# derekmetcalf/epnn

Hardware: AMD Instinct MI355X
Metric: atoms/sec (inference), QM9-sized batch (higher is better)
Workload: dtype f32; 1 GPU; qm9_like_b1024_N29; molecules_per_gpu=1024, atoms_per_gpu=18521, N=29, pairs_under_cutoff_per_gpu=72439, entry=epnn_forward_xyz_dev (coordinates in HBM), weights=decay_model_weights, parallelism=molecule-sharded x1, batches_in_flight_per_gpu=8

## Files before the change

epnn_amd/csrc/epnn_wave.hip.h:

```cpp
#pragma once
#include <type_traits>

#include "epnn_common.h"
#include "epnn_frontend.hip.h"

struct WaveArgs {
    const float *wpack;
    const float *xin;
    const float *Q;
    const int4 *wblk;
    const int *row_off;
    const int *pi, *pj, *psym;
    float *pe, *pwi, *pwj;
    float *q_out;
    float *h_out;
    int *status;
    int N, T, nx, A;
    const float *h_in;
    const float *q_in;
    const float *nm_in;
    float *gx;
    int lds_words;
    const float *xyz;
    double cut2;
// ... 112 lines not shown
#ifndef EPNN_SPLIT_VALU
__device__ __forceinline__ void w16_split3(const float (&v)[8], u32x4 &p1, u32x4 &p2, u32x4 &p3) {
    const w16_u32x2 I = w16_ident();
    f32x4 x0 = {v[0], v[1], v[2], v[3]}, x1 = {v[4], v[5], v[6], v[7]};
    p1 = w16_pack_hi(x0, x1);
    x0 = w16_rem(I, p1[0], p1[1], x0); x1 = w16_rem(I, p1[2], p1[3], x1);
    p2 = w16_pack_hi(x0, x1);
    x0 = w16_rem(I, p2[0], p2[1], x0); x1 = w16_rem(I, p2[2], p2[3], x1);
    p3 = w16_pack_hi(x0, x1);
}
#else
__device__ __forceinline__ void w16_split3(const float (&v)[8], u32x4 &p1, u32x4 &p2, u32x4 &p3) {
    float r1[8], r2[8];
#pragma unroll
    for (int s = 0; s < 8; ++s) {
        r1[s] = v[s] - __uint_as_float(__float_as_uint(v[s]) & 0xffff0000u);
        r2[s] = r1[s] - __uint_as_float(__float_as_uint(r1[s]) & 0xffff0000u);
    }
#pragma unroll
    for (int j = 0; j < 4; ++j) {
        p1[j] = __builtin_amdgcn_perm(__float_as_uint(v[2 * j + 1]), __float_as_uint(v[2 * j]), 0x07060302u);
        p2[j] = __builtin_amdgcn_perm(__float_as_uint(r1[2 * j + 1]), __float_as_uint(r1[2 * j]), 0x07060302u);
        p3[j] = __builtin_amdgcn_perm(__float_as_uint(r2[2 * j + 1]), __float_as_uint(r2[2 * j]), 0x07060302u);
    }
}
#endif
__device__ __forceinline__ void w16_mm_bf(const u32x4 (&w)[2][3], u32x4 z1, u32x4 z2, u32x4 z3, f32x4 (&d)[2]) {
#pragma unroll
    for (int rb = 0; rb < 2; ++rb) {
        d[rb] = w16_mfma_bf(w[rb][0], z3, d[rb]);
        d[rb] = w16_mfma_bf(w[rb][1], z2, d[rb]);
        d[rb] = w16_mfma_bf(w[rb][2], z1, d[rb]);
        d[rb] = w16_mfma_bf(w[rb][0], z2, d[rb]);
        d[rb] = w16_mfma_bf(w[rb][1], z1, d[rb]);
        d[rb] = w16_mfma_bf(w[rb][0], z1, d[rb]);
    }
}
#define W16_LDB(dst, off)                                                                                       \
    _Pragma("unroll") for (int rb_ = 0; rb_ < 2; ++rb_)                                                         \
        _Pragma("unroll") for (int pc_ = 0; pc_ < 3; ++pc_)                                                     \
            (dst)[rb_][pc_] = reinterpret_cast<const u32x4 *>(wp + (size_t)(unsigned)(off))[(rb_ * 3 + pc_) * 64 + lane];
__device__ __forceinline__ void w16_split3k16(f32x4 x, w16_u32x2 &p1, w16_u32x2 &p2, w16_u32x2 &p3) {
    const w16_u32x2 I = w16_ident();
    p1 = w16_pack_hi2(x);
    x = w16_rem(I, p1[0], p1[1], x);
    p2 = w16_pack_hi2(x);
    x = w16_rem(I, p2[0], p2[1], x);
    p3 = w16_pack_hi2(x);
}
__device__ __forceinline__ void w16_mm_bfk16(const w16_u32x2 (&w)[2][3], const w16_u32x2 (&z)[3], f32x4 (&d)[2]) {
#pragma unroll
    for (int rb = 0; rb < 2; ++rb) {
        d[rb] = w16_rem(w[rb][0], z[2][0], z[2][1], d[rb]);
        d[rb] = w16_rem(w[rb][1], z[1][0], z[1][1], d[rb]);
        d[rb] = w16_rem(w[rb][2], z[0][0], z[0][1], d[rb]);
        d[rb] = w16_rem(w[rb][0], z[1][0], z[1][1], d[rb]);
        d[rb] = w16_rem(w[rb][1], z[0][0], z[0][1], d[rb]);
        d[rb] = w16_rem(w[rb][0], z[0][0], z[0][1], d[rb]);
    }
}
#define W16_LDB16(dst, off)                                                                                     \
    _Pragma("unroll") for (int rb_ = 0; rb_ < 2; ++rb_)                                                         \
        _Pragma("unroll") for (int pc_ = 0; pc_ < 3; ++pc_)                                                     \
            (dst)[rb_][pc_] = reinterpret_cast<const w16_u32x2 *>(wp + (size_t)(unsigned)(off))[(rb_ * 3 + pc_) * 64 + lane];
__device__ __forceinline__ f32x4 w16_relu(f32x4 v) {
    return f32x4{fmaxf(v[0], 0.f), fmaxf(v[1], 0.f), fmaxf(v[2], 0.f), fmaxf(v[3], 0.f)};
}
__device__ __forceinline__ float w16_sumq(float v) {
    const auto a = __builtin_amdgcn_permlane16_swap(__float_as_uint(v), __float_as_uint(v), false, false);
    const float s = __uint_as_float(a[0]) + __uint_as_float(a[1]);
    const auto b = __builtin_amdgcn_permlane32_swap(__float_as_uint(s), __float_as_uint(s), false, false);
    return __uint_as_float(b[0]) + __uint_as_float(b[1]);
}
__device__ __forceinline__ f32x4 w16_ld(const float *p) { return *reinterpret_cast<const f32x4 *>(p); }
__device__ __forceinline__ void w16_st(float *p, f32x4 v) { *reinterpret_cast<f32x4 *>(p) = v; }

typedef __attribute__((address_space(3))) const f32x4 w16_lds_cf4;
typedef __attribute__((address_space(3))) const unsigned short w16_lds_cu16;
__device__ __forceinline__ unsigned w16_lds_addr(const void *p) { return (unsigned)(size_t)(__attribute__((address_space(3))) const char *)p; }
__device__ __forceinline__ f32x4 w16_lds_ld4(unsigned a) { return *(w16_lds_cf4 *)(size_t)a; }
__device__ __forceinline__ unsigned w16_lds_ldu16(unsigned a) { return *(w16_lds_cu16 *)(size_t)a; }
typedef __attribute__((address_space(3))) const unsigned w16_lds_cu32;
__device__ __forceinline__ unsigned w16_lds_ldu32(unsigned a) { return *(w16_lds_cu32 *)(size_t)a; }
__device__ __forceinline__ f32x2 w16_lo(f32x4 v) { return __builtin_shufflevector(v, v, 0, 1); }
__device__ __forceinline__ f32x2 w16_hi(f32x4 v) { return __builtin_shufflevector(v, v, 2, 3); }
__device__ __forceinline__ f32x4 w16_cat(f32x2 a, f32x2 b) { return __builtin_shufflevector(a, b, 0, 1, 2, 3); }

#define W16_LDX(dst, off, nrb, cnt, stride, s0)                                                                   \
    _Pragma("unroll") for (int rb_ = 0; rb_ < (nrb); ++rb_) {                                                     \
        const f32x4 *fp_ = reinterpret_cast<const f32x4 *>(wp + (size_t)(unsigned)(off)) +                        \
                           (size_t)(unsigned)((rb_ * ((stride) / 4) + (s0) / 4) * 64 + lane);                     \
        _Pragma("unroll") for (int g_ = 0; g_ < (cnt) / 4; ++g_) {                                                \
            const f32x4 v_ = fp_[g_ * 64];                                                                        \
            (dst)[rb_][4 * g_] = v_[0]; (dst)[rb_][4 * g_ + 1] = v_[1]; (dst)[rb_][4 * g_ + 2] = v_[2]; (dst)[rb_][4 * g_ + 3] = v_[3]; \
        }                                                                                                         \
    }
#define W16_LD(dst, off, nrb, steps) W16_LDX(dst, off, nrb, steps, steps, 0)

template <int NRB, int S>
__device__ __forceinline__ void w16_mm(const float (&w)[NRB][S], const float (&in)[S], f32x4 (&d)[NRB]) {
#pragma unroll
    for (int rb = 0; rb < NRB; ++rb)
#pragma unroll
        for (int s = 0; s < S; ++s) d[rb] = w16_mfma(w[rb][s], in[s], d[rb]);
}
template <int NRB, int S, int SKIP>
__device__ __forceinline__ void w16_mm_skip(const float (&w)[NRB][S], const float (&in)[S], f32x4 (&d)[NRB], bool skip) {
#pragma unroll
    for (int rb = 0; rb < NRB; ++rb)
#pragma unroll
        for (int s = 0; s < S; ++s) {
            if (s == SKIP) {
                if (!skip) d[rb] = w16_mfma(w[rb][s], in[s], d[rb]);
            } else {
                d[rb] = w16_mfma(w[rb][s], in[s], d[rb]);
            }
        }
}
template <int NRB>
__device__ __forceinline__ void w16_feed(const f32x4 (&a)[NRB], float (&in)[4 * NRB]) {
#pragma unroll
    for (int s = 0; s < 4 * NRB; ++s) in[s] = a[s >> 2][s & 3];
}

#ifdef EPNN_G_F32
#define W16_G_BF 0
#else
#define W16_G_BF 1
#endif
#define W16_G_DECL                                                                                                        \
    constexpr bool GB = FRONT && W16_G_BF;                                                                                \
    w16_u32x2 gwb[2][3];                                                                                                  \
    auto g_mm = [&](const float (&e)[KE], f32x4 (&d)[2]) {                  \
        if constexpr (GB) {                                                                                               \
            w16_u32x2 z[3];                                                                                               \
            w16_split3k16(f32x4{e[0], e[1], e[2], e[3]}, z[0], z[1], z[2]);                                               \
            w16_mm_bfk16(gwb, z, d);                                                                                      \
        } else {                                                                                                          \
            w16_mm<2, KE>(gw, e, d);                                                                                      \
        }                                                                                                                 \
    }
#define GW_LD(off, offb)                                                                                                  \
    do {                                                                                                                  \
        if constexpr (GB) {                                                                                               \
            W16_LDB16(gwb, offb);                                                                                         \
        } else { W16_LD(gw, off, 2, KE); }                                                                                \
    } while (0)
template <bool GNN, bool EPN, bool FRONT, int NRU = 2>
__global__ __launch_bounds__(64, EPNN_WAVES_PER_SIMD) void k_wave_forward(WaveArgs A, WaveIndex X) {
    extern __shared__ __attribute__((aligned(16))) float sm[];
    const int lane = threadIdx.x, q = lane >> 4, n16 = lane & 15;
    const int c = lane & 31, hh = lane >> 5;
    if (!FRONT && (*A.status & EPNN_ST_PAIR_OVERFLOW)) return;
    const int4 wb = A.wblk[blockIdx.x];
    const int b = wb.x, a0 = wb.y, n = wb.z;
    if (A.prio_n > 0 && n >= A.prio_n) __builtin_amdgcn_s_setprio(3);
    const int p0 = FRONT ? wb.w : A.row_off[a0];
    int np = FRONT ? 0 : A.row_off[a0 + n] - p0;
    const int nx = A.nx;
    const bool xs3 = nx + 3 <= 4 * (EPNN_XS - 1);
    const float *wp = A.wpack;
    int nstamp = 0;
    (void)nstamp;
#ifdef EPNN_STAMPS
    const unsigned long long rt0 = __builtin_amdgcn_s_memrealtime();
#endif
    WAVE_STAMP();
    const bool two = n > 16;
    const int m1 = two ? n - 16 : 16, C1 = 16 / m1;
    const int copy1 = n16 / m1;
    const int col1 = 16 + n16 % m1;
    const bool cat0 = n16 < n, cat1 = two && copy1 < C1;
    const bool own1 = cat1 && copy1 == 0;

    const int ia0 = a0 + min(n16, n - 1), ia1 = a0 + (two ? col1 : 0);
    float cxyz[3] = {0.f, 0.f, 0.f};
    if (FRONT) {
        const float *xr = A.xyz + 3 * (size_t)(a0 + min(c, n - 1));
        cxyz[0] = xr[0]; cxyz[1] = xr[1]; cxyz[2] = xr[2];
    }
    float nmv0 = 1.f, nmv1 = 1.f, qa0, qa1, Qb = 0.f;
    if (A.nm_in) { nmv0 = A.nm_in[ia0]; nmv1 = A.nm_in[ia1]; }
    if (A.q_in) { qa0 = A.q_in[ia0]; qa1 = A.q_in[ia1]; }
    else Qb = A.Q[b];
    float xv0[EPNN_XS], xv1[EPNN_XS];
#pragma unroll
    for (int s = 0; s < EPNN_XS; ++s) {
        const int xi = min(max(4 * s + q - 1, 0), A.nx - 1);
        xv0[s] = A.xin[(size_t)ia0 * A.nx + xi];
        xv1[s] = A.xin[(size_t)ia1 * A.nx + xi];
    }
    f32x4 hk0[3], hk1[3];
#pragma unroll
    for (int rb = 0; rb < 3; ++rb) { hk0[rb] = w16_splat(0.f); hk1[rb] = w16_splat(0.f); }
    const bool have_h = A.h_in != nullptr;
    if (have_h) {
#pragma unroll
        for (int rb = 0; rb < 3; ++rb) {
            const f32x4 v0 = w16_ld(A.h_in + (size_t)ia0 * EPNN_EDIM + 16 * rb + 4 * q), v1 = w16_ld(A.h_in + (size_t)ia1 * EPNN_EDIM + 16 * rb + 4 * q);
            if (cat0) hk0[rb] = v0;
            if (cat1) hk1[rb] = v1;
        }
    }
    WAVE_FENCE();

    unsigned short *eij = reinterpret_cast<unsigned short *>(sm);
    const int eij_n = FRONT ? n * (n - 1) / 2 : np;
    const int o_r = EPN ? ((((eij_n + 1) >> 1) + 3) & ~3) : 0;
    float *Rl = sm + o_r;
    const int o_x = o_r + n * EPNN_PST;
    unsigned short *pm = reinterpret_cast<unsigned short *>(sm + o_x);
    const int NPM = ((n + 9) & ~3) + 2;
    float *Pl = sm + o_x;
    constexpr int DMS = 36;
    float *Dm = sm + o_x + n * EPNN_PST;
    const int o_gg = o_x + ((((n * NPM + 1) >> 1) + 3) & ~3);
    const int grows_g = (A.lds_words - o_gg) / EPNN_PST - 1;
    float *Gl = sm + o_gg;
    const unsigned zent = 4u * (unsigned)o_gg;
    auto pm_ent = [&](int slot) -> unsigned short {
        return (unsigned short)(slot < grows_g ? 4u * (unsigned)(o_gg + (slot + 1) * EPNN_PST) : (1u | (unsigned)slot << 1));
    };
    int glds = min(np, grows_g);
    bool gover = np > glds;
    int ngt = (np + 31) >> 5;

    double *xs = reinterpret_cast<double *>(Rl);
    if (FRONT) {
        if (hh == 0 && c < n) {
            xs[3 * c + 0] = (double)cxyz[0];
            xs[3 * c + 1] = (double)cxyz[1];
            xs[3 * c + 2] = (double)cxyz[2];
        }
        wave_sync_lds();
        WAVE_STAMP_I();
    }
    constexpr int KE = FRONT ? EPNN_ER / 4 : 12;
    int ptl = 0;
    const unsigned pt_top = w16_lds_addr(sm + A.lds_words) + 16u * (unsigned)q;
    auto load_e1 = [&](int slot, float (&e)[KE]) {
        const int sl = slot < np ? slot : 0;
        if (FRONT) {
            f32x4 v;
            if (sl < ptl) v = w16_lds_ld4(pt_top - 64u * (unsigned)(sl + 1));
            else v = w16_ld(A.pt + (size_t)(p0 + sl) * EPNN_ER + 4 * q);
            e[0] = v[0]; e[1] = v[1]; e[2] = v[2]; e[3] = v[3];
        } else {
            const float *r = A.pe + (size_t)(p0 + sl) * EPNN_EDIM + 12 * q;
#pragma unroll
            for (int k = 0; k < 3; ++k) {
                const f32x4 v = w16_ld(r + 4 * k);
                e[(4 * k) % KE] = v[0]; e[(4 * k + 1) % KE] = v[1]; e[(4 * k + 2) % KE] = v[2]; e[(4 * k + 3) % KE] = v[3];
            }
        }
    };
    auto load_e = [&](int gt, float (&e0)[KE], float (&e1)[KE]) {
        load_e1(gt * 32 + n16, e0);
        load_e1(gt * 32 + 16 + n16, e1);
    };
    float gw[2][KE], ge0[KE], ge1[KE];
    W16_G_DECL;
    GW_LD(FRONT ? X.g[0].we16 : (GNN ? X.g[0].we : X.e[0].we), X.g[0].we16b);
    if (GNN && !FRONT && ngt > 0) load_e(0, ge0, ge1);
    WAVE_FENCE();

    if (GNN)
        for (int i = lane; i < (n * NPM + 1) >> 1; i += 64) reinterpret_cast<unsigned *>(pm)[i] = zent | zent << 16;
    wave_sync_lds();
    if (FRONT) {
        WAVE_STAMP_I();
        int base = 0;
        const double cx = (double)cxyz[0], cy = (double)cxyz[1], cz = (double)cxyz[2];
        for (int i0 = 0; i0 + 1 < n; i0 += 4) {
            const int iA = i0 + hh, iB = min(i0 + 2 + hh, n - 1);
            const double dA = wave_dist2c(xs, iA, cx, cy, cz), dB = wave_dist2c(xs, iB, cx, cy, cz);
            const bool nearA = c > iA && c < n && dA < A.cut2;
            const bool nearB = i0 + 3 < n && c > iB && c < n && dB < A.cut2;
            const unsigned long long balA = __ballot(nearA), balB = __ballot(nearB);
            const unsigned loA = (unsigned)balA, hiA = (unsigned)(balA >> 32), loB = (unsigned)balB, hiB = (unsigned)(balB >> 32);
            const int baseB = base + __popc(loA) + __popc(hiA);
            if (nearA) {
                const int slot = base + (hh ? __popc(loA) : 0) + __popc((hh ? hiA : loA) & ((1u << c) - 1u));
                eij[slot] = (unsigned short)(iA | (c << 8));
                pm[c * NPM + iA] = pm_ent(slot);
                pm[iA * NPM + c] = pm_ent(slot);
            }
            if (nearB) {
                const int slot = baseB + (hh ? __popc(loB) : 0) + __popc((hh ? hiB : loB) & ((1u << c) - 1u));
                eij[slot] = (unsigned short)(iB | (c << 8));
                pm[c * NPM + iB] = pm_ent(slot);
                pm[iB * NPM + c] = pm_ent(slot);
            }
            base = baseB + __popc(loB) + __popc(hiB);
        }
        np = base;
        glds = min(np, grows_g);
        gover = np > glds;
        ngt = (np + 31) >> 5;
        ptl = min(np, max(0, A.lds_words - max(o_gg + (glds + 1) * EPNN_PST, o_x + n * (EPNN_PST + DMS))) / EPNN_ER);
        wave_sync_lds();
        WAVE_STAMP_I();
        for (int s0 = 0; s0 < np; s0 += 64) {
            if (s0 + lane < np) {
                const int ij = eij[s0 + lane];
                const double D = wave_dist(xs, ij & 0xFF, ij >> 8);
                if (wave_near(A.flip, A.nflip, D)) eij[s0 + lane] = (unsigned short)(ij | 0x80);
                const double tt = D * A.tab_inv_h;
                const int i0 = min(max((int)tt - 1, 0), A.tab_n - 4);
                const float u = (float)(tt - (double)i0);
                const float um1 = u - 1.f, um2 = u - 2.f, um3 = u - 3.f;
                const float w0 = -(um1 * um2 * um3) * (1.f / 6.f), w1 = (u * um2 * um3) * 0.5f;
                const float w2 = -(u * um1 * um3) * 0.5f, w3 = (u * um1 * um2) * (1.f / 6.f);
                const float *trow = A.etab + (size_t)i0 * EPNN_ER;
                f32x4 tv[4][EPNN_ER / 4];
#pragma unroll
                for (int k = 0; k < 4; ++k)
#pragma unroll
                    for (int g = 0; g < EPNN_ER / 4; ++g) tv[k][g] = w16_ld(trow + k * EPNN_ER + 4 * g);
                f32x4 v[EPNN_ER / 4];
#pragma unroll
                for (int g = 0; g < EPNN_ER / 4; ++g) v[g] = w0 * tv[0][g] + w1 * tv[1][g] + w2 * tv[2][g] + w3 * tv[3][g];
                if (s0 + lane < ptl) {
                    float *prow = sm + A.lds_words - (size_t)(s0 + lane + 1) * EPNN_ER;
#pragma unroll
                    for (int g = 0; g < EPNN_ER / 4; ++g) w16_st(prow + 4 * g, v[g]);
                }
                asm volatile("" ::: "memory");
                if (s0 + lane >= ptl) {
                    float *prow = A.pt + (size_t)(p0 + s0 + lane) * EPNN_ER;
#pragma unroll
                    for (int g = 0; g < EPNN_ER / 4; ++g) w16_st(prow + 4 * g, v[g]);
                }
            }
        }
        wave_sync_all();
        WAVE_STAMP_I();
        if (ngt > 0) load_e(0, ge0, ge1);
    } else {
        if (GNN)
            for (int p = lane; p < np; p += 64) {
                const int li = A.pi[p0 + p] - a0, lj = A.pj[p0 + p] - a0;
                pm[li * NPM + lj] = pm_ent(p);
                if (A.psym[p0 + p]) pm[lj * NPM + li] = pm_ent(p);
            }
        if (EPN)
            for (int p = lane; p < np; p += 64) {
                const int li = A.pi[p0 + p] - a0, lj = A.pj[p0 + p] - a0;
                eij[p] = (unsigned short)(li | (lj << 8));
            }
    }
    if (GNN)
        for (int i = lane; i < EPNN_PST; i += 64) Gl[i] = 0.f;
    wave_sync_lds();
    const float nm0 = cat0 ? nmv0 : 0.f, nm1 = cat1 ? nmv1 : 0.f;
    float xq0[EPNN_XS], xq1[EPNN_XS];
    {
        if (!A.q_in) qa0 = qa1 = Qb / (float)n;
        const float qv0 = cat0 ? qa0 : 0.f, qv1 = cat1 ? qa1 : 0.f;
#pragma unroll
        for (int s = 0; s < EPNN_XS; ++s) {
            const int phi = 4 * s + q;
            float v0 = 0.f, v1 = 0.f;
            if (phi == 0) { v0 = nm0; v1 = nm1; }
            else if (phi <= nx) { v0 = cat0 ? xv0[s] : 0.f; v1 = cat1 ? xv1[s] : 0.f; }
            else if (phi == nx + 1) { v0 = qv0; v1 = qv1; }
            else if (phi == nx + 2) { v0 = cat0 ? 1.f : 0.f; v1 = cat1 ? 1.f : 0.f; }
            xq0[s] = v0;
            xq1[s] = v1;
        }
    }

#ifdef EPNN_CHAIN_F32
    constexpr bool CHB = false;
#else
    constexpr bool CHB = NRU == 2 && GNN;
#endif
    u32x4 Bp0[3], Bp1[3];
    w16_u32x2 xqb0[3], xqb1[3];
    float qc0 = 0.f, qc1 = 0.f;
    auto xq_charge = [&]() {
        if (q != 0) return;
        const float a0_ = __uint_as_float(__float_as_uint(qc0) & 0xffff0000u), r0_ = qc0 - a0_;
// ... 412 lines not shown
                W16_LD(pb, X.g[t + 1].w2, 2, 8);
#else
                W16_LDB(pb, X.g[t + 1].w2b);
#endif
                vec2(X.g[t + 1].b2, b2v);
#pragma unroll
                for (int rb = 0; rb < 2; ++rb) { U0[rb] = nm0 * cu[rb]; U1[rb] = nm1 * cu[rb]; }
                w16_mm_bf(wh, Bp0[0], Bp0[1], Bp0[2], U0);
                if (two) w16_mm_bf(wh, Bp1[0], Bp1[1], Bp1[2], U1);
                wave_sync_all();
                if (t < 2) WAVE_STAMP();
              }
            } else
            if (!lastg) {
                float wa[2][KU + EPNN_XS], wb[2][KU + EPNN_XS], in0[KU + EPNN_XS], in1[KU + EPNN_XS];
                W16_LD(wa, M.pwi, 2, KU + EPNN_XS);
                WAVE_FENCE();
                gtiles();
                if (t < 2) WAVE_STAMP();
#pragma unroll
                for (int s = 0; s < KU; ++s) { in0[s] = B0[s >> 2][s & 3]; in1[s] = B1[s >> 2][s & 3]; }
#pragma unroll
                for (int s = 0; s < EPNN_XS; ++s) { in0[KU + s] = xq0[s]; in1[KU + s] = xq1[s]; }
                W16_LD(wb, M.pwj, 2, KU + EPNN_XS);
                float wu[NRU][KU];
                f32x4 cu[NRU];
                if constexpr (NRU == 2) { W16_LD(wu, M.pu1, NRU, KU); }
                vecu(M.cu3, cu);
                WAVE_FENCE();
#pragma unroll
                for (int rb = 0; rb < 2; ++rb) { P0[rb] = w16_splat(0.f); P1[rb] = w16_splat(0.f); }
                w16_mm_skip<2, KU + EPNN_XS, KU - 1 + EPNN_XS>(wa, in0, P0, xs3);
                if (two) w16_mm_skip<2, KU + EPNN_XS, KU - 1 + EPNN_XS>(wa, in1, P1, xs3);
                f32x4 r0[2] = {w16_splat(0.f), w16_splat(0.f)}, r1[2] = {w16_splat(0.f), w16_splat(0.f)};
                w16_mm_skip<2, KU + EPNN_XS, KU - 1 + EPNN_XS>(wb, in0, r0, xs3);
                if (two) w16_mm_skip<2, KU + EPNN_XS, KU - 1 + EPNN_XS>(wb, in1, r1, xs3);
                if (cat0) { w16_st(Rl + n16 * EPNN_PST + fo, r0[0]); w16_st(Rl + n16 * EPNN_PST + 16 + fo, r0[1]); }
                if (own1) { w16_st(Rl + col1 * EPNN_PST + fo, r1[0]); w16_st(Rl + col1 * EPNN_PST + 16 + fo, r1[1]); }
                if constexpr (NRU != 2) { W16_LD(wu, M.pu1, NRU, KU); }
#ifdef EPNN_SWEEP_F32
                W16_LD(pb, X.g[t + 1].w2, 2, 8);
#else
                W16_LDB(pb, X.g[t + 1].w2b);
#endif
                vec2(X.g[t + 1].b2, b2v);
                WAVE_FENCE();
                float bin0[KU], bin1[KU];
                w16_feed<NRU>(B0, bin0);
                w16_feed<NRU>(B1, bin1);
#pragma unroll
                for (int rb = 0; rb < NRU; ++rb) { U0[rb] = nm0 * cu[rb]; U1[rb] = nm1 * cu[rb]; }
                w16_mm<NRU, KU>(wu, bin0, U0);
                if (two) w16_mm<NRU, KU>(wu, bin1, U1);
                wave_sync_all();
                if (t < 2) WAVE_STAMP();
            }
        }
        if (!FOLD || A.h_out) {
            float w[3][KU], bin0[KU], bin1[KU];
            W16_LD(w, X.u3, 3, KU);
            f32x4 bv[3];
#pragma unroll
            for (int rb = 0; rb < 3; ++rb) bv[rb] = w16_ld(wp + X.bu3 + 16 * rb + fo);
            WAVE_FENCE();
            w16_feed<NRU>(B0, bin0);
            w16_feed<NRU>(B1, bin1);
#pragma unroll
            for (int rb = 0; rb < 3; ++rb) { hk0[rb] = nm0 * bv[rb]; hk1[rb] = nm1 * bv[rb]; }
            w16_mm<3, KU>(w, bin0, hk0);
            if (two) w16_mm<3, KU>(w, bin1, hk1);
        }
        if (A.h_out) {
#pragma unroll
            for (int rb = 0; rb < 3; ++rb) {
                if (cat0) w16_st(A.h_out + (size_t)(a0 + n16) * EPNN_EDIM + 16 * rb + fo, hk0[rb]);
                if (own1) w16_st(A.h_out + (size_t)(a0 + col1) * EPNN_EDIM + 16 * rb + fo, hk1[rb]);
            }
        }
    }

    WAVE_STAMP();
    if (EPN) {
        wave_sync_lds();
        for (int i = lane; i < n * DMS; i += 64) Dm[i] = 0.f;
        if (FRONT && ptl < np) {
            const int pte = min(np, (A.lds_words - (o_x + n * (EPNN_PST + DMS))) / EPNN_ER);
            for (int i = lane; i < (pte - ptl) * (EPNN_ER / 4); i += 64) {
                const int r = ptl + (i >> 2), k = i & 3;
                w16_st(sm + A.lds_words - (size_t)(r + 1) * EPNN_ER + 4 * k, w16_ld(A.pt + (size_t)(p0 + r) * EPNN_ER + 4 * k));
            }
            ptl = max(ptl, pte);
            asm volatile("s_waitcnt vmcnt(0)" ::: "memory");
        }
        wave_sync_lds();
        const int qs = (nx + 1) >> 2, ql = (nx + 1) & 3;
#pragma unroll 1
        for (int t = 0; t < Te; ++t) {
            const WaveEpnPack &M = X.e[t];
            if constexpr (CHB && FOLD) {
                u32x4 wh[2][3];
                w16_u32x2 wx[2][3];
                W16_LDB(wh, M.wifhb);
                W16_LDB16(wx, M.wifxb);
                WAVE_FENCE();
                f32x4 d0[2] = {w16_splat(0.f), w16_splat(0.f)}, d1[2] = {w16_splat(0.f), w16_splat(0.f)};
                w16_mm_bf(wh, Bp0[0], Bp0[1], Bp0[2], d0);
                if (two) w16_mm_bf(wh, Bp1[0], Bp1[1], Bp1[2], d1);
                xq_mm(wx, d0, d1);
                W16_LDB(wh, M.wjfhb);
                W16_LDB16(wx, M.wjfxb);
                if (cat0) { w16_st(Pl + n16 * EPNN_PST + fo, d0[0]); w16_st(Pl + n16 * EPNN_PST + 16 + fo, d0[1]); }
                if (own1) { w16_st(Pl + col1 * EPNN_PST + fo, d1[0]); w16_st(Pl + col1 * EPNN_PST + 16 + fo, d1[1]); }
                d0[0] = w16_splat(0.f); d0[1] = w16_splat(0.f); d1[0] = w16_splat(0.f); d1[1] = w16_splat(0.f);
                w16_mm_bf(wh, Bp0[0], Bp0[1], Bp0[2], d0);
                if (two) w16_mm_bf(wh, Bp1[0], Bp1[1], Bp1[2], d1);
                xq_mm(wx, d0, d1);
                if (cat0) { w16_st(Rl + n16 * EPNN_PST + fo, d0[0]); w16_st(Rl + n16 * EPNN_PST + 16 + fo, d0[1]); }
                if (own1) { w16_st(Rl + col1 * EPNN_PST + fo, d1[0]); w16_st(Rl + col1 * EPNN_PST + 16 + fo, d1[1]); }
            } else {
                constexpr int KS = FOLD ? KU + EPNN_XS : EPNN_XS + 12;
                constexpr int SK = FOLD ? KU - 1 + EPNN_XS : EPNN_XS - 1;
                float wa[2][KS], wb[2][KS], in0[KS], in1[KS];
                if (FOLD) {
#pragma unroll
                    for (int s = 0; s < KU; ++s) { in0[s] = B0[s >> 2][s & 3]; in1[s] = B1[s >> 2][s & 3]; }
#pragma unroll
                    for (int s = 0; s < EPNN_XS; ++s) { in0[KU + s] = xq0[s]; in1[KU + s] = xq1[s]; }
                } else {
#pragma unroll
                    for (int s = 0; s < EPNN_XS; ++s) { in0[s] = xq0[s]; in1[s] = xq1[s]; }
#pragma unroll
                    for (int s = 0; s < 12; ++s) { in0[EPNN_XS + s] = hk0[s >> 2][s & 3]; in1[EPNN_XS + s] = hk1[s >> 2][s & 3]; }
                }
                W16_LD(wa, FOLD ? M.wif : M.wi, 2, KS);
                W16_LD(wb, FOLD ? M.wjf : M.wj, 2, KS);
                WAVE_FENCE();
                f32x4 d0[2] = {w16_splat(0.f), w16_splat(0.f)}, d1[2] = {w16_splat(0.f), w16_splat(0.f)};
                w16_mm_skip<2, KS, SK>(wa, in0, d0, xs3);
                if (two) w16_mm_skip<2, KS, SK>(wa, in1, d1, xs3);
                if (cat0) { w16_st(Pl + n16 * EPNN_PST + fo, d0[0]); w16_st(Pl + n16 * EPNN_PST + 16 + fo, d0[1]); }
                if (own1) { w16_st(Pl + col1 * EPNN_PST + fo, d1[0]); w16_st(Pl + col1 * EPNN_PST + 16 + fo, d1[1]); }
                d0[0] = w16_splat(0.f); d0[1] = w16_splat(0.f); d1[0] = w16_splat(0.f); d1[1] = w16_splat(0.f);
                w16_mm_skip<2, KS, SK>(wb, in0, d0, xs3);
                if (two) w16_mm_skip<2, KS, SK>(wb, in1, d1, xs3);
                if (cat0) { w16_st(Rl + n16 * EPNN_PST + fo, d0[0]); w16_st(Rl + n16 * EPNN_PST + 16 + fo, d0[1]); }
                if (own1) { w16_st(Rl + col1 * EPNN_PST + fo, d1[0]); w16_st(Rl + col1 * EPNN_PST + 16 + fo, d1[1]); }
            }
#ifdef EPNN_SWEEP_F32
            float pb[2][8];
            W16_LD(pb, M.w2, 2, 8);
#else
            u32x4 pb[2][3];
            W16_LDB(pb, M.w2b);
#endif
            f32x4 b2v[2], w3[2];
            vec2(M.b2, b2v);
            vec2(M.w3, w3);
            wave_sync_all();
            if (t < 2) WAVE_STAMP();
            {
                const int nblk = (np + 15) >> 4;
                struct Rec { int ij; float wi, wj; };
                struct Rows { float e[KE]; f32x4 pi_[2], rj_[2], pj_[2], ri_[2]; };
                auto load_rec = [&](int blk, Rec &r_) {
                    const int sl = blk * 16 + n16 < np ? blk * 16 + n16 : 0;
                    r_.ij = eij[sl];
                    if (FRONT) {
                        r_.wi = r_.wj = (r_.ij & 0x80) ? 1.f : 0.f;
                        r_.ij &= 0xFF7F;
                    } else {
                        r_.wi = A.pwi[p0 + sl];
                        r_.wj = A.pwj[p0 + sl];
                    }
                };
                auto load_rows = [&](int blk, const Rec &r_, Rows &w_) {
                    const int sl = blk * 16 + n16 < np ? blk * 16 + n16 : 0;
                    const int li = r_.ij & 0xFF, lj = r_.ij >> 8;
                    load_e1(sl, w_.e);
#pragma unroll
                    for (int rb = 0; rb < 2; ++rb) {
                        w_.pi_[rb] = w16_ld(Pl + li * EPNN_PST + 16 * rb + fo);
                        w_.rj_[rb] = w16_ld(Rl + lj * EPNN_PST + 16 * rb + fo);
                        w_.pj_[rb] = w16_ld(Pl + lj * EPNN_PST + 16 * rb + fo);
                        w_.ri_[rb] = w16_ld(Rl + li * EPNN_PST + 16 * rb + fo);
                    }
                };
                auto block = [&](int blk, const Rec &r_, const Rows &w_) {
                    const bool valid = blk * 16 + n16 < np;
                    const int li = r_.ij & 0xFF, lj = r_.ij >> 8;
                    f32x4 g[2] = {w16_splat(0.f), w16_splat(0.f)};
                    g_mm(w_.e, g);
                    const f32x4 ua = w16_relu((g[0] + w_.pi_[0]) + w_.rj_[0]), ub = w16_relu((g[1] + w_.pi_[1]) + w_.rj_[1]);
                    const f32x4 va = w16_relu((g[0] + w_.pj_[0]) + w_.ri_[0]), vb = w16_relu((g[1] + w_.pj_[1]) + w_.ri_[1]);
                    const float zu[8] = {ua[0], ua[1], ua[2], ua[3], ub[0], ub[1], ub[2], ub[3]};
                    const float zv[8] = {va[0], va[1], va[2], va[3], vb[0], vb[1], vb[2], vb[3]};
                    f32x4 au[2] = {b2v[0], b2v[1]}, av[2] = {b2v[0], b2v[1]};
#ifdef EPNN_SWEEP_F32
                    WAVE_FENCE();
                    w16_mm<2, 8>(pb, zu, au);
                    w16_mm<2, 8>(pb, zv, av);
#else
                    u32x4 zu1, zu2, zu3, zv1, zv2, zv3;
                    w16_split3(zu, zu1, zu2, zu3);
                    w16_split3(zv, zv1, zv2, zv3);
                    WAVE_FENCE();
                    w16_mm_bf(pb, zu1, zu2, zu3, au);
                    w16_mm_bf(pb, zv1, zv2, zv3, av);
#endif
                    WAVE_FENCE();
                    float fd = 0.f;
#pragma unroll
                    for (int rb = 0; rb < 2; ++rb) {
                        const f32x4 t = w16_relu(au[rb]) - w16_relu(av[rb]);
#pragma unroll
                        for (int r = 0; r < 4; ++r) fd = fmaf(w3[rb][r], t[r], fd);
                    }
                    const float d = 0.5f * w16_sumq(fd);
                    const float wq = q == 0 ? r_.wi : r_.wj;
                    const int to = q == 0 ? li : lj, from = q == 0 ? lj : li;
                    if (q < 2 && valid && wq != 0.f) Dm[to * DMS + ((from & 3) << 3) + (from >> 2)] = q == 0 ? wq * d : -(wq * d);
                };
                if (nblk > 0) {
                    Rec r0, r1;
                    Rows w0, w1;
                    load_rec(0, r0);
                    load_rec(min(1, nblk - 1), r1);
                    load_rows(0, r0, w0);
                    int blk = 0;
#pragma unroll 1
                    for (; blk + 1 < nblk; blk += 2) {
                        Rec r2, r3;
                        load_rows(blk + 1, r1, w1);
                        load_rec(min(blk + 2, nblk - 1), r2);
                        WAVE_FENCE();
                        block(blk, r0, w0);
                        load_rows(min(blk + 2, nblk - 1), r2, w0);
                        load_rec(min(blk + 3, nblk - 1), r3);
                        WAVE_FENCE();
                        block(blk + 1, r1, w1);
                        r0 = r2;
                        r1 = r3;
                    }
                    if (blk < nblk) block(blk, r0, w0);
                }
            }
            wave_sync_lds();
            if (t + 1 < Te) { GW_LD(FRONT ? X.e[t + 1].we16 : X.e[t + 1].we, X.e[t + 1].we16b); }
            WAVE_FENCE();
            if (t < 2) WAVE_STAMP();
            {
                float dq0 = 0.f, dq1 = 0.f;
                const unsigned r0a = w16_lds_addr(Dm + (cat0 ? n16 : 0) * DMS) + 32u * (unsigned)q, r1a = w16_lds_addr(Dm + (cat1 ? col1 : 0) * DMS) + 32u * (unsigned)q;
                const f32x4 u0 = w16_lds_ld4(r0a), u1 = w16_lds_ld4(r1a);
#pragma unroll
                for (int k = 0; k < 4; ++k) { dq0 += u0[k]; dq1 += u1[k]; }
                if (two) {
                    const f32x4 v0 = w16_lds_ld4(r0a + 16u), v1 = w16_lds_ld4(r1a + 16u);
#pragma unroll
                    for (int k = 0; k < 4; ++k) { dq0 += v0[k]; dq1 += v1[k]; }
                }
                dq0 = w16_sumq(dq0);
                dq1 = w16_sumq(dq1);
                if constexpr (CHB && FOLD) {
                    qc0 += cat0 ? dq0 : 0.f;
                    qc1 += cat1 ? dq1 : 0.f;
                    xq_charge();
                } else {
#pragma unroll
                    for (int s = 0; s < EPNN_XS; ++s)
                        if (s == qs && q == ql) { xq0[s] += cat0 ? dq0 : 0.f; xq1[s] += cat1 ? dq1 : 0.f; }
                }
            }
            wave_sync_lds();
            if (t < 2) WAVE_STAMP();
        }
        if constexpr (CHB && FOLD) {
            if (q == 0) {
                if (cat0) A.q_out[a0 + n16] = qc0;
                if (own1) A.q_out[a0 + col1] = qc1;
            }
        } else {
#pragma unroll
            for (int s = 0; s < EPNN_XS; ++s)
                if (s == qs && q == ql) {
                    if (cat0) A.q_out[a0 + n16] = xq0[s];
                    if (own1) A.q_out[a0 + col1] = xq1[s];
                }
        }
    }
    if (FRONT && A.handoff && lane == 0) wave_handoff(A, np);
    WAVE_STAMP();
#ifdef EPNN_STAMPS
    if (lane == 0 && A.stamps) {
        A.stamps[(size_t)blockIdx.x * 64 + 61] = (unsigned long long)__builtin_amdgcn_s_getreg(4 | (0 << 6) | (31 << 11)) |
                                                 ((unsigned long long)__builtin_amdgcn_s_getreg(20 | (0 << 6) | (3 << 11)) << 32);
        A.stamps[(size_t)blockIdx.x * 64 + 59] = rt0;
        A.stamps[(size_t)blockIdx.x * 64 + 60] = __builtin_amdgcn_s_memrealtime();
        A.stamps[(size_t)blockIdx.x * 64 + 62] = (unsigned long long)nstamp;
        A.stamps[(size_t)blockIdx.x * 64 + 63] = ((unsigned long long)n << 32) | (unsigned)np;
    }
#endif
    (void)Tg;
}
```

Baseline: 342.8 million atoms/s.

## Precompute packed pair records in LDS and relocate edge-message buffers

Before the edge-message loop, each pair's i/j indices, LDS row offsets, Dm scatter offsets and validity flag are packed into a 32-bit record stored in LDS. The inner loop then decodes these with bit-field extracts and direct LDS addressing instead of reloading the 16-bit eij index and recomputing offsets. The R/P/Dm buffers move to sit after the record array, and the LDS budget calculation is updated to match. This trims per-block integer work and scalar loads, at the cost of a serial packing pass with barriers and a larger Dm stride.

```diff
diff --git a/epnn_amd/csrc/epnn_wave.hip.h b/epnn_amd/csrc/epnn_wave.hip.h
--- a/epnn_amd/csrc/epnn_wave.hip.h
+++ b/epnn_amd/csrc/epnn_wave.hip.h
@@ -218,6 +218,8 @@
 __device__ __forceinline__ unsigned w16_lds_ldu16(unsigned a) { return *(w16_lds_cu16 *)(size_t)a; }
 typedef __attribute__((address_space(3))) const unsigned w16_lds_cu32;
 __device__ __forceinline__ unsigned w16_lds_ldu32(unsigned a) { return *(w16_lds_cu32 *)(size_t)a; }
+__device__ __forceinline__ f32x4 w16_lds_ld4k(unsigned a, int k) { return ((w16_lds_cf4 *)(size_t)a)[k]; }
+__device__ __forceinline__ void w16_lds_st1(unsigned a, float v) { *(__attribute__((address_space(3))) float *)(size_t)a = v; }
 __device__ __forceinline__ f32x2 w16_lo(f32x4 v) { return __builtin_shufflevector(v, v, 0, 1); }
 __device__ __forceinline__ f32x2 w16_hi(f32x4 v) { return __builtin_shufflevector(v, v, 2, 3); }
 __device__ __forceinline__ f32x4 w16_cat(f32x2 a, f32x2 b) { return __builtin_shufflevector(a, b, 0, 1, 2, 3); }
@@ -347,9 +349,8 @@
     const int o_x = o_r + n * EPNN_PST;
     unsigned short *pm = reinterpret_cast<unsigned short *>(sm + o_x);
     const int NPM = ((n + 9) & ~3) + 2;
-    float *Pl = sm + o_x;
-    constexpr int DMS = 36;
-    float *Dm = sm + o_x + n * EPNN_PST;
+    constexpr int DMS = EPNN_PST;
+    auto epn_words = [&](int pairs) { return ((pairs + 15) & ~15) + n * (2 * EPNN_PST + DMS); };
     const int o_gg = o_x + ((((n * NPM + 1) >> 1) + 3) & ~3);
     const int grows_g = (A.lds_words - o_gg) / EPNN_PST - 1;
     float *Gl = sm + o_gg;
@@ -433,7 +434,7 @@
         glds = min(np, grows_g);
         gover = np > glds;
         ngt = (np + 31) >> 5;
-        ptl = min(np, max(0, A.lds_words - max(o_gg + (glds + 1) * EPNN_PST, o_x + n * (EPNN_PST + DMS))) / EPNN_ER);
+        ptl = min(np, max(0, A.lds_words - max(o_gg + (glds + 1) * EPNN_PST, epn_words(np))) / EPNN_ER);
         wave_sync_lds();
         WAVE_STAMP_I();
         for (int s0 = 0; s0 < np; s0 += 64) {
@@ -1012,9 +1013,25 @@
     WAVE_STAMP();
     if (EPN) {
         wave_sync_lds();
+        const int np16 = (np + 15) & ~15;
+        unsigned *rec = reinterpret_cast<unsigned *>(sm);
+        for (int s0 = (np16 - 1) & ~63; s0 >= 0; s0 -= 64) {
+            const int p = s0 + lane;
+            unsigned r = 0x80000000u;
+            if (p < np) {
+                const unsigned ij = eij[p];
+                const unsigned li = ij & (FRONT ? 0x7Fu : 0xFFu), lj = ij >> 8;
+                r = 9u * li | (((li & 3u) << 3) + (li >> 2)) << 9 | 9u * lj << 16 | (((lj & 3u) << 3) + (lj >> 2)) << 25;
+                if (FRONT && !(ij & 0x80u)) r |= 0x80000000u;
+            }
+            wave_sync_lds();
+            if (p < np16) rec[p] = r;
+            wave_sync_lds();
+        }
+        float *Re = sm + np16, *Pl = Re + n * EPNN_PST, *Dm = Pl + n * EPNN_PST;
         for (int i = lane; i < n * DMS; i += 64) Dm[i] = 0.f;
         if (FRONT && ptl < np) {
-            const int pte = min(np, (A.lds_words - (o_x + n * (EPNN_PST + DMS))) / EPNN_ER);
+            const int pte = min(np, (A.lds_words - epn_words(np)) / EPNN_ER);
             for (int i = lane; i < (pte - ptl) * (EPNN_ER / 4); i += 64) {
                 const int r = ptl + (i >> 2), k = i & 3;
                 w16_st(sm + A.lds_words - (size_t)(r + 1) * EPNN_ER + 4 * k, w16_ld(A.pt + (size_t)(p0 + r) * EPNN_ER + 4 * k));
@@ -1023,6 +1040,10 @@
             asm volatile("s_waitcnt vmcnt(0)" ::: "memory");
         }
         wave_sync_lds();
+        const unsigned reb = w16_lds_addr(Re) + 16u * (unsigned)q, plb = w16_lds_addr(Pl) + 16u * (unsigned)q;
+        const unsigned dmb = w16_lds_addr(Dm), recb = w16_lds_addr(rec) + 4u * (unsigned)n16;
+        const unsigned sh_to = q == 0 ? 0u : 16u, sh_from = q == 0 ? 25u : 9u;
+        const float sgn = q == 0 ? 1.f : -1.f;
         const int qs = (nx + 1) >> 2, ql = (nx + 1) & 3;
 #pragma unroll 1
         for (int t = 0; t < Te; ++t) {
@@ -1045,8 +1066,8 @@
                 w16_mm_bf(wh, Bp0[0], Bp0[1], Bp0[2], d0);
                 if (two) w16_mm_bf(wh, Bp1[0], Bp1[1], Bp1[2], d1);
                 xq_mm(wx, d0, d1);
-                if (cat0) { w16_st(Rl + n16 * EPNN_PST + fo, d0[0]); w16_st(Rl + n16 * EPNN_PST + 16 + fo, d0[1]); }
-                if (own1) { w16_st(Rl + col1 * EPNN_PST + fo, d1[0]); w16_st(Rl + col1 * EPNN_PST + 16 + fo, d1[1]); }
+                if (cat0) { w16_st(Re + n16 * EPNN_PST + fo, d0[0]); w16_st(Re + n16 * EPNN_PST + 16 + fo, d0[1]); }
+                if (own1) { w16_st(Re + col1 * EPNN_PST + fo, d1[0]); w16_st(Re + col1 * EPNN_PST + 16 + fo, d1[1]); }
             } else {
                 constexpr int KS = FOLD ? KU + EPNN_XS : EPNN_XS + 12;
                 constexpr int SK = FOLD ? KU - 1 + EPNN_XS : EPNN_XS - 1;
@@ -1073,8 +1094,8 @@
                 d0[0] = w16_splat(0.f); d0[1] = w16_splat(0.f); d1[0] = w16_splat(0.f); d1[1] = w16_splat(0.f);
                 w16_mm_skip<2, KS, SK>(wb, in0, d0, xs3);
                 if (two) w16_mm_skip<2, KS, SK>(wb, in1, d1, xs3);
-                if (cat0) { w16_st(Rl + n16 * EPNN_PST + fo, d0[0]); w16_st(Rl + n16 * EPNN_PST + 16 + fo, d0[1]); }
-                if (own1) { w16_st(Rl + col1 * EPNN_PST + fo, d1[0]); w16_st(Rl + col1 * EPNN_PST + 16 + fo, d1[1]); }
+                if (cat0) { w16_st(Re + n16 * EPNN_PST + fo, d0[0]); w16_st(Re + n16 * EPNN_PST + 16 + fo, d0[1]); }
+                if (own1) { w16_st(Re + col1 * EPNN_PST + fo, d1[0]); w16_st(Re + col1 * EPNN_PST + 16 + fo, d1[1]); }
             }
 #ifdef EPNN_SWEEP_F32
             float pb[2][8];
@@ -1089,35 +1110,27 @@
             wave_sync_all();
             if (t < 2) WAVE_STAMP();
             {
-                const int nblk = (np + 15) >> 4;
-                struct Rec { int ij; float wi, wj; };
+                const int nblk = np16 >> 4;
+                struct Rec { unsigned rec; float w; };
                 struct Rows { float e[KE]; f32x4 pi_[2], rj_[2], pj_[2], ri_[2]; };
                 auto load_rec = [&](int blk, Rec &r_) {
-                    const int sl = blk * 16 + n16 < np ? blk * 16 + n16 : 0;
-                    r_.ij = eij[sl];
-                    if (FRONT) {
-                        r_.wi = r_.wj = (r_.ij & 0x80) ? 1.f : 0.f;
-                        r_.ij &= 0xFF7F;
-                    } else {
-                        r_.wi = A.pwi[p0 + sl];
-                        r_.wj = A.pwj[p0 + sl];
+                    r_.rec = w16_lds_ldu32(recb + 64u * (unsigned)blk);
+                    if (FRONT) r_.w = 1.f;
+                    else r_.w = (q == 0 ? A.pwi : A.pwj)[p0 + (blk * 16 + n16 < np ? blk * 16 + n16 : 0)];
+                };
+                auto load_rows = [&](int blk, const Rec &r_, Rows &w_) {
+                    const unsigned oi = (r_.rec & 0x1ffu) << 4, oj = __builtin_amdgcn_ubfe(r_.rec, 16u, 9u) << 4;
+                    const unsigned api = plb + oi, arj = reb + oj, apj = plb + oj, ari = reb + oi;
+                    load_e1(blk * 16 + n16, w_.e);
+#pragma unroll
+                    for (int rb = 0; rb < 2; ++rb) {
+                        w_.pi_[rb] = w16_lds_ld4k(api, 4 * rb);
+                        w_.rj_[rb] = w16_lds_ld4k(arj, 4 * rb);
+                        w_.pj_[rb] = w16_lds_ld4k(apj, 4 * rb);
+                        w_.ri_[rb] = w16_lds_ld4k(ari, 4 * rb);
                     }
                 };
-                auto load_rows = [&](int blk, const Rec &r_, Rows &w_) {
-                    const int sl = blk * 16 + n16 < np ? blk * 16 + n16 : 0;
-                    const int li = r_.ij & 0xFF, lj = r_.ij >> 8;
-                    load_e1(sl, w_.e);
-#pragma unroll
-                    for (int rb = 0; rb < 2; ++rb) {
-                        w_.pi_[rb] = w16_ld(Pl + li * EPNN_PST + 16 * rb + fo);
-                        w_.rj_[rb] = w16_ld(Rl + lj * EPNN_PST + 16 * rb + fo);
-                        w_.pj_[rb] = w16_ld(Pl + lj * EPNN_PST + 16 * rb + fo);
-                        w_.ri_[rb] = w16_ld(Rl + li * EPNN_PST + 16 * rb + fo);
-                    }
-                };
-                auto block = [&](int blk, const Rec &r_, const Rows &w_) {
-                    const bool valid = blk * 16 + n16 < np;
-                    const int li = r_.ij & 0xFF, lj = r_.ij >> 8;
+                auto block = [&](const Rec &r_, const Rows &w_) {
                     f32x4 g[2] = {w16_splat(0.f), w16_splat(0.f)};
                     g_mm(w_.e, g);
                     const f32x4 ua = w16_relu((g[0] + w_.pi_[0]) + w_.rj_[0]), ub = w16_relu((g[1] + w_.pi_[1]) + w_.rj_[1]);
@@ -1146,9 +1159,8 @@
                         for (int r = 0; r < 4; ++r) fd = fmaf(w3[rb][r], t[r], fd);
                     }
                     const float d = 0.5f * w16_sumq(fd);
-                    const float wq = q == 0 ? r_.wi : r_.wj;
-                    const int to = q == 0 ? li : lj, from = q == 0 ? lj : li;
-                    if (q < 2 && valid && wq != 0.f) Dm[to * DMS + ((from & 3) << 3) + (from >> 2)] = q == 0 ? wq * d : -(wq * d);
+                    const unsigned da = dmb + (__builtin_amdgcn_ubfe(r_.rec, sh_to, 9u) << 4) + (__builtin_amdgcn_ubfe(r_.rec, sh_from, 5u) << 2);
+                    if (q < 2 && (int)r_.rec >= 0 && (FRONT || r_.w != 0.f)) w16_lds_st1(da, FRONT ? sgn * d : sgn * (r_.w * d));
                 };
                 if (nblk > 0) {
                     Rec r0, r1;
@@ -1163,15 +1175,15 @@
                         load_rows(blk + 1, r1, w1);
                         load_rec(min(blk + 2, nblk - 1), r2);
                         WAVE_FENCE();
-                        block(blk, r0, w0);
+                        block(r0, w0);
                         load_rows(min(blk + 2, nblk - 1), r2, w0);
                         load_rec(min(blk + 3, nblk - 1), r3);
                         WAVE_FENCE();
-                        block(blk + 1, r1, w1);
+                        block(r1, w1);
                         r0 = r2;
                         r1 = r3;
                     }
-                    if (blk < nblk) block(blk, r0, w0);
+                    if (blk < nblk) block(r0, w0);
                 }
             }
             wave_sync_lds();
```

Result: no change. 345.0 million atoms/s, median of 6 (+0.6%).

## Precompute per-pair bf16 split edge features and LDS addresses into a table

Applied to the files above, without the earlier changes.

Before the per-layer pair sweep, each pair's edge features are split once into bf16 pieces and stored in LDS. The same table entry also holds the packed row addresses and the Dm store address, so the sweep loop no longer repeats the split, index decode and address arithmetic on every layer. Pairs that do not fit in the spare LDS fall back to the old path. The cost is an extra setup pass and more LDS use, and the result depends on LDS headroom and pointer packing into 16 bits.

```diff
diff --git a/epnn_amd/csrc/epnn_wave.hip.h b/epnn_amd/csrc/epnn_wave.hip.h
--- a/epnn_amd/csrc/epnn_wave.hip.h
+++ b/epnn_amd/csrc/epnn_wave.hip.h
@@ -218,6 +218,11 @@
 __device__ __forceinline__ unsigned w16_lds_ldu16(unsigned a) { return *(w16_lds_cu16 *)(size_t)a; }
 typedef __attribute__((address_space(3))) const unsigned w16_lds_cu32;
 __device__ __forceinline__ unsigned w16_lds_ldu32(unsigned a) { return *(w16_lds_cu32 *)(size_t)a; }
+typedef __attribute__((address_space(3))) u32x4 w16_lds_u4;
+typedef __attribute__((address_space(3))) float w16_lds_f1;
+__device__ __forceinline__ u32x4 w16_lds_ldu4(unsigned a) { return *(const w16_lds_u4 *)(size_t)a; }
+__device__ __forceinline__ void w16_lds_stu4(unsigned a, u32x4 v) { *(w16_lds_u4 *)(size_t)a = v; }
+__device__ __forceinline__ void w16_lds_stf(unsigned a, float v) { *(w16_lds_f1 *)(size_t)a = v; }
 __device__ __forceinline__ f32x2 w16_lo(f32x4 v) { return __builtin_shufflevector(v, v, 0, 1); }
 __device__ __forceinline__ f32x2 w16_hi(f32x4 v) { return __builtin_shufflevector(v, v, 2, 3); }
 __device__ __forceinline__ f32x4 w16_cat(f32x2 a, f32x2 b) { return __builtin_shufflevector(a, b, 0, 1, 2, 3); }
@@ -1023,6 +1028,34 @@
             asm volatile("s_waitcnt vmcnt(0)" ::: "memory");
         }
         wave_sync_lds();
+        constexpr bool TB = GB && NRU == 2;
+        int ktab = 0;
+        const unsigned tb_off = 4u * EPNN_ER * (unsigned)ptl;
+        if constexpr (TB) {
+            const int kfit = min(ptl, max(0, A.lds_words - (o_x + n * (EPNN_PST + DMS)) - EPNN_ER * ptl) / 16);
+            ktab = kfit >= np ? np : (kfit & ~15);
+            const unsigned pl_a = w16_lds_addr(Pl) + 16u * (unsigned)q, dm_a = w16_lds_addr(Dm);
+            for (int s0 = 0; s0 < ktab; s0 += 16) {
+                const bool ok = s0 + n16 < ktab;
+                const int sl = ok ? s0 + n16 : 0;
+                const unsigned ra = pt_top - 64u * (unsigned)(sl + 1);
+                const f32x4 v = w16_lds_ld4(ra);
+                const unsigned ij = eij[sl];
+                w16_u32x2 z[3];
+                w16_split3k16(v, z[0], z[1], z[2]);
+                const unsigned li = ij & 0x7Fu, lj = ij >> 8;
+                const unsigned to = q == 0 ? li : lj, from = q == 0 ? lj : li;
+                const unsigned rows = (pl_a + 4u * EPNN_PST * li) | (pl_a + 4u * EPNN_PST * lj) << 16;
+                const unsigned st = (q < 2 && (ij & 0x80u)) ? dm_a + 4u * (to * DMS + ((from & 3u) << 3) + (from >> 2)) : ~0u;
+                asm volatile("" ::: "memory");
+                if (ok) {
+                    w16_lds_stu4(ra, u32x4{z[0][0], z[0][1], z[1][0], z[1][1]});
+                    w16_lds_stu4(ra - tb_off, u32x4{z[2][0], z[2][1], rows, st});
+                }
+                asm volatile("" ::: "memory");
+            }
+            wave_sync_lds();
+        }
         const int qs = (nx + 1) >> 2, ql = (nx + 1) & 3;
 #pragma unroll 1
         for (int t = 0; t < Te; ++t) {
@@ -1092,8 +1125,9 @@
                 const int nblk = (np + 15) >> 4;
                 struct Rec { int ij; float wi, wj; };
                 struct Rows { float e[KE]; f32x4 pi_[2], rj_[2], pj_[2], ri_[2]; };
+                const int sl_pad = ktab < np ? ktab : 0;
                 auto load_rec = [&](int blk, Rec &r_) {
-                    const int sl = blk * 16 + n16 < np ? blk * 16 + n16 : 0;
+                    const int sl = blk * 16 + n16 < np ? blk * 16 + n16 : sl_pad;
                     r_.ij = eij[sl];
                     if (FRONT) {
                         r_.wi = r_.wj = (r_.ij & 0x80) ? 1.f : 0.f;
@@ -1104,7 +1138,7 @@
                     }
                 };
                 auto load_rows = [&](int blk, const Rec &r_, Rows &w_) {
-                    const int sl = blk * 16 + n16 < np ? blk * 16 + n16 : 0;
+                    const int sl = blk * 16 + n16 < np ? blk * 16 + n16 : sl_pad;
                     const int li = r_.ij & 0xFF, lj = r_.ij >> 8;
                     load_e1(sl, w_.e);
 #pragma unroll
@@ -1115,11 +1149,7 @@
                         w_.ri_[rb] = w16_ld(Rl + li * EPNN_PST + 16 * rb + fo);
                     }
                 };
-                auto block = [&](int blk, const Rec &r_, const Rows &w_) {
-                    const bool valid = blk * 16 + n16 < np;
-                    const int li = r_.ij & 0xFF, lj = r_.ij >> 8;
-                    f32x4 g[2] = {w16_splat(0.f), w16_splat(0.f)};
-                    g_mm(w_.e, g);
+                auto pair_d = [&](const f32x4 (&g)[2], const auto &w_) -> float {
                     const f32x4 ua = w16_relu((g[0] + w_.pi_[0]) + w_.rj_[0]), ub = w16_relu((g[1] + w_.pi_[1]) + w_.rj_[1]);
                     const f32x4 va = w16_relu((g[0] + w_.pj_[0]) + w_.ri_[0]), vb = w16_relu((g[1] + w_.pj_[1]) + w_.ri_[1]);
                     const float zu[8] = {ua[0], ua[1], ua[2], ua[3], ub[0], ub[1], ub[2], ub[3]};
@@ -1145,18 +1175,78 @@
 #pragma unroll
                         for (int r = 0; r < 4; ++r) fd = fmaf(w3[rb][r], t[r], fd);
                     }
-                    const float d = 0.5f * w16_sumq(fd);
+                    return 0.5f * w16_sumq(fd);
+                };
+                auto block = [&](int blk, const Rec &r_, const Rows &w_) {
+                    const bool valid = blk * 16 + n16 < np;
+                    const int li = r_.ij & 0xFF, lj = r_.ij >> 8;
+                    f32x4 g[2] = {w16_splat(0.f), w16_splat(0.f)};
+                    g_mm(w_.e, g);
+                    const float d = pair_d(g, w_);
                     const float wq = q == 0 ? r_.wi : r_.wj;
                     const int to = q == 0 ? li : lj, from = q == 0 ? lj : li;
                     if (q < 2 && valid && wq != 0.f) Dm[to * DMS + ((from & 3) << 3) + (from >> 2)] = q == 0 ? wq * d : -(wq * d);
                 };
-                if (nblk > 0) {
+                const int nbt = (ktab + 15) >> 4;
+                if constexpr (TB) {
+                    struct RecT { u32x4 a, b; };
+                    struct RowsT { f32x4 pi_[2], rj_[2], pj_[2], ri_[2]; };
+                    const unsigned pr_d = 4u * EPNN_PST * (unsigned)n;
+                    auto load_rec_t = [&](int blk, RecT &r_) {
+                        const int sl = blk * 16 + n16 < ktab ? blk * 16 + n16 : 0;
+                        const unsigned ra = pt_top - 64u * (unsigned)(sl + 1);
+                        r_.a = w16_lds_ldu4(ra);
+                        r_.b = w16_lds_ldu4(ra - tb_off);
+                    };
+                    auto load_rows_t = [&](const RecT &r_, RowsT &w_) {
+                        const unsigned pi = r_.b[2] & 0xFFFFu, pj = r_.b[2] >> 16, ri = pi - pr_d, rj = pj - pr_d;
+#pragma unroll
+                        for (int rb = 0; rb < 2; ++rb) {
+                            w_.pi_[rb] = w16_lds_ld4(pi + 64u * rb);
+                            w_.rj_[rb] = w16_lds_ld4(rj + 64u * rb);
+                            w_.pj_[rb] = w16_lds_ld4(pj + 64u * rb);
+                            w_.ri_[rb] = w16_lds_ld4(ri + 64u * rb);
+                        }
+                    };
+                    auto block_t = [&](int blk, const RecT &r_, const RowsT &w_) {
+                        const bool valid = blk * 16 + n16 < ktab;
+                        f32x4 g[2] = {w16_splat(0.f), w16_splat(0.f)};
+                        const w16_u32x2 z[3] = {{r_.a[0], r_.a[1]}, {r_.a[2], r_.a[3]}, {r_.b[0], r_.b[1]}};
+                        w16_mm_bfk16(gwb, z, g);
+                        const float d = pair_d(g, w_);
+                        if (valid && r_.b[3] != ~0u) w16_lds_stf(r_.b[3], q == 0 ? d : -d);
+                    };
+                    if (nbt > 0) {
+                        RecT r0, r1;
+                        RowsT w0, w1;
+                        load_rec_t(0, r0);
+                        load_rec_t(min(1, nbt - 1), r1);
+                        load_rows_t(r0, w0);
+                        int blk = 0;
+#pragma unroll 1
+                        for (; blk + 1 < nbt; blk += 2) {
+                            RecT r2, r3;
+                            load_rows_t(r1, w1);
+                            load_rec_t(min(blk + 2, nbt - 1), r2);
+                            WAVE_FENCE();
+                            block_t(blk, r0, w0);
+                            load_rows_t(r2, w0);
+                            load_rec_t(min(blk + 3, nbt - 1), r3);
+                            WAVE_FENCE();
+                            block_t(blk + 1, r1, w1);
+                            r0 = r2;
+                            r1 = r3;
+                        }
+                        if (blk < nbt) block_t(blk, r0, w0);
+                    }
+                }
+                if (nbt < nblk) {
                     Rec r0, r1;
                     Rows w0, w1;
-                    load_rec(0, r0);
-                    load_rec(min(1, nblk - 1), r1);
-                    load_rows(0, r0, w0);
-                    int blk = 0;
+                    load_rec(nbt, r0);
+                    load_rec(min(nbt + 1, nblk - 1), r1);
+                    load_rows(nbt, r0, w0);
+                    int blk = nbt;
 #pragma unroll 1
                     for (; blk + 1 < nblk; blk += 2) {
                         Rec r2, r3;
```

New measurement: 343.6 million atoms/s before, 348.3 million atoms/s after, median of 6. 1.01x the previous value.
